# hannesweisbach/channelcoding

Hardware: AMD Instinct MI355X
Metric: decoded frames/sec (coded bits/sec = value x 255), BCH(255,231) min-sum, batch=2^20 (higher is better)
Workload: dtype f32

## Files before the change

channelcoding_amd/csrc/cc_internal.hpp:

```cpp
#pragma once
#include <hip/hip_runtime.h>

#include <cstdint>
#include <memory>
#include <mutex>
#include <string>
#include <vector>

#include "../../include/channelcoding_amd.h"
#include "galois.hpp"

namespace ccamd {

struct MinSumGeometry {
  int W = 64, C = 4, frames_per_wave = 1, KW = 1;
};

struct MinSumParams {
  int n, K, KW;
  int variant;
  int stop_rule;
  unsigned iterations;
  float alpha_f;
  float beta_f;
// ... 111 lines not shown
  bool scms;
  int np = 0;
  int gap[4] = {0, 0, 0, 0};
};
const DiagGeometry *diag_geometry(const CodeTables &t);
std::vector<uint16_t> build_diag_table(const CodeTables &t, int D, int W, int np = 0, const int *gap = nullptr);
size_t minsum_diag_lds_bytes(const DiagGeometry &g);
MinSumParams minsum_params(const cc_code *code);
bool minsum_shortcuts_enabled();
bool minsum_diag_supported(const cc_code *code);
int launch_minsum_diag_compact(const cc_code *code, uint32_t *d_ctl, uint32_t *d_pool, unsigned cap, const float *d_llr,
                               uint8_t *d_hard, uint16_t *d_iters, int32_t *d_status, hipStream_t stream);
std::string minsum_diag_name(const cc_code *code);
int launch_minsum_diag(const cc_code *code, const MinSumParams &p, const float *d_llr, const uint16_t *d_er,
                       const uint32_t *d_er_off, uint8_t *d_hard, float *d_L, uint16_t *d_iters, int32_t *d_status,
                       size_t B, hipStream_t stream);
bool algebraic_long_needed(const cc_code *code, bool erasures);
int launch_algebraic_long(const cc_code *code, bool float_in, const void *d_in, const uint16_t *d_er,
                          const uint32_t *d_er_off, uint8_t *d_out, int32_t *d_nerr, int32_t *d_status, size_t B,
                          hipStream_t stream);
int launch_algebraic(const cc_code *code, bool float_in, const void *d_in, const uint16_t *d_er,
                     const uint32_t *d_er_off, uint8_t *d_out, int32_t *d_nerr, int32_t *d_status, size_t B,
                     hipStream_t stream);
bool algebraic_chunk_supported(const cc_code *code, bool erasures);
int launch_algebraic_chunk(const cc_code *code, bool float_in, const void *d_in, const uint16_t *d_er,
                           const uint32_t *d_er_off, uint8_t *d_out, int32_t *d_nerr, int32_t *d_status, size_t B,
                           hipStream_t stream, int il = 1);
int launch_chase(const cc_code *code, const float *d_llr, unsigned p, uint8_t *d_out, int32_t *d_nerr, float *d_metric,
                 int32_t *d_status, size_t B, hipStream_t stream);
int chase_frames_per_wave(const cc_code *code, unsigned p, bool soft);
int launch_chase_soft(const cc_code *code, const float *d_llr, unsigned p, float beta, uint8_t *d_out, float *d_ext,
                      int32_t *d_nerr, float *d_metric, int32_t *d_status, size_t B, hipStream_t stream);
int launch_gmd(const cc_code *code, const uint8_t *d_words, const float *d_rel, unsigned m, uint8_t *d_out, int32_t *d_nerr,
               float *d_metric, int32_t *d_status, size_t B, hipStream_t stream);
bool bitslice_supported(const cc_code *code);
int launch_bitslice_syndromes(const cc_code *code, bool float_in, const void *d_in, uint8_t *d_out, uint8_t *d_synd, size_t B,
                              hipStream_t stream, int il = 1);
bool bitslice_encode_supported(const cc_code *code);
int launch_bitslice_encode(const cc_code *code, const uint8_t *d_msg, uint8_t *d_cw, size_t B, hipStream_t stream, int il = 1);
int launch_bitslice_chien(const void *d_lamp, void *d_masks, size_t B, bool long_locators, hipStream_t stream);
int launch_bitslice_roots_transpose(const void *d_masks, void *d_rootsT, size_t B, hipStream_t stream);
constexpr uint32_t kLogZero = 512;
int launch_chunk_bm(const cc_code *code, const uint8_t *d_synd, const uint16_t *d_er, const uint32_t *d_er_off,
                    uint16_t *d_llg, uint16_t *d_meta, unsigned long long *d_mask, uint8_t *d_lamp, int ncoef,
                    uint32_t *d_nleft, int32_t *d_nerr, int32_t *d_status, size_t B, hipStream_t stream);
int algebraic_route(const cc_code *code, size_t B, bool erasures);
bool planes_small_call(const cc_code *code, size_t B);
int launch_pgz_erasures(const cc_code *code, const uint8_t *d_in, const uint16_t *d_er, const uint32_t *d_er_off,
                        uint8_t *d_out, int32_t *d_nerr, int32_t *d_status, size_t B, hipStream_t stream);
constexpr int diag_variant_part(int variant, int parts) {
  const int order = variant == CC_ALG_MS ? 0 : variant == CC_ALG_NMS ? 1 : variant == CC_ALG_OMS ? 2
                  : variant == CC_ALG_SCMS2 ? 3 : variant == CC_ALG_SCMS1 ? 4 : 5;
  return order % parts;
}

int launch_wide_correct(const cc_code *code, const uint16_t *d_in, const uint16_t *d_er, const uint32_t *d_off,
                        uint16_t *d_out, int32_t *d_nerr, int32_t *d_status, size_t B, hipStream_t stream);
int launch_wide_pgz_erasures(const cc_code *code, const uint16_t *d_in, const uint16_t *d_er, const uint32_t *d_off,
                        uint16_t *d_out, int32_t *d_nerr, int32_t *d_status, size_t B, hipStream_t stream);
int launch_wide_encode(const cc_code *code, const uint16_t *d_msg, uint16_t *d_cw, size_t B, hipStream_t stream);
int launch_wide_extract(const cc_code *code, const uint16_t *d_cw, uint16_t *d_msg, size_t B, hipStream_t stream);
std::vector<uint8_t> build_parity_table(const Field &f, const CodeTables &t);
int launch_encode(const cc_code *code, const uint8_t *d_msg, uint8_t *d_cw, size_t B, hipStream_t stream);
int launch_encode_bits(const cc_code *code, const uint8_t *d_msg, uint8_t *d_cw, size_t B, hipStream_t stream);
int launch_extract(const cc_code *code, const uint8_t *d_cw, uint8_t *d_msg, size_t B, hipStream_t stream);
int launch_pack_bits(const void *d_sym, int width, size_t n, uint8_t *d_packed, size_t B, hipStream_t stream);
int launch_unpack_bits(const uint8_t *d_packed, size_t n, void *d_sym, int width, size_t B, hipStream_t stream);
bool packed_native_supported(const cc_code *code, size_t B);
int launch_packed_correct(const cc_code *code, const uint8_t *d_in, uint8_t *d_out, int32_t *d_nerr, int32_t *d_status,
                          size_t B, hipStream_t stream);
bool packed_long_supported(const cc_code *code, size_t B);
int launch_packed_long_correct(const cc_code *code, const uint8_t *d_in, uint8_t *d_out, int32_t *d_nerr, int32_t *d_status,
                               size_t B, hipStream_t stream);
bool packed_encode_native(const cc_code *code);
bool packed_extract_native(const cc_code *code);
int launch_packed_encode(const cc_code *code, const uint8_t *d_msg, uint8_t *d_cw, size_t B, hipStream_t stream);
int launch_packed_extract(const cc_code *code, const uint8_t *d_cw, uint8_t *d_msg, size_t B, hipStream_t stream);
constexpr size_t kInterleaveMax = 256;
constexpr size_t kInterleaveNativeMax = 16;
int launch_interleave(const void *d_in, int width, size_t n, size_t I, void *d_out, size_t B, bool to_interleaved,
                      hipStream_t stream);
bool interleaved_native_supported(const cc_code *code, size_t B, size_t I, bool erasures);
bool interleaved_encode_native(const cc_code *code, size_t I);
bool interleaved_extract_native(const cc_code *code, size_t I);
int launch_interleaved_extract(const cc_code *code, const void *d_cw, void *d_msg, size_t B, size_t I, hipStream_t stream);
int mc_run(cc_code *code, double ebno_db, uint64_t seed, uint64_t first_frame, size_t frames, int random_codewords,
           uint64_t *d_counters, hipStream_t stream);
int mc_run_chase(cc_code *code, unsigned p, double ebno_db, uint64_t seed, uint64_t first_frame, size_t frames,
                 int random_codewords, uint64_t *d_counters, hipStream_t stream);
int mc_run_gmd(cc_code *code, unsigned m, double ebno_db, uint64_t seed, uint64_t first_frame, size_t frames,
               int random_codewords, uint64_t *d_counters, hipStream_t stream);
int mc_awgn_symbols(cc_code *code, double ebno_db, uint64_t seed, uint64_t first_frame, size_t frames, int random_codewords,
                    uint8_t *d_words, float *d_rel, uint8_t *d_sent, hipStream_t stream);
int mc_awgn(cc_code *code, double ebno_db, uint64_t seed, uint64_t first_frame, size_t frames, int random_codewords,
            float *d_llr, uint8_t *d_sent, hipStream_t stream);
int mc_run_discrete(cc_code *code, double p_error, double p_erasure, uint64_t seed, uint64_t first_frame, size_t frames,
                    int random_codewords, uint64_t *d_counters, hipStream_t stream);
int mc_discrete(cc_code *code, double p_error, double p_erasure, uint64_t seed, uint64_t first_frame, size_t frames,
                int random_codewords, uint8_t *d_recv, uint16_t *d_erasures, uint32_t *d_erasure_offsets,
                uint8_t *d_sent, hipStream_t stream);
int mc_run_burst(cc_code *code, const cc_burst_channel &ch, uint64_t seed, uint64_t first_frame, size_t frames,
                 int random_codewords, uint64_t *d_counters, hipStream_t stream);
int mc_burst(cc_code *code, const cc_burst_channel &ch, uint64_t seed, uint64_t first_frame, size_t frames,
             int random_codewords, uint8_t *d_recv, uint8_t *d_sent, uint8_t *d_state, hipStream_t stream);
int mc_run_burst_erasure(cc_code *code, const cc_burst_channel &ch, const cc_burst_detector &det, uint64_t seed,
                         uint64_t first_frame, size_t frames, int random_codewords, uint64_t *d_counters,
// ... 23 lines not shown
```

channelcoding_amd/csrc/minsum_diag.hip:

```cpp
#include "minsum_diag_impl.hpp"

#include <algorithm>
#include <cstdlib>

namespace ccamd {

using DiagLaunch = int (*)(const cc_code *, const MinSumParams &, const float *, const uint16_t *, const uint32_t *,
                           uint8_t *, float *, uint16_t *, int32_t *, size_t, hipStream_t);
#define CC_PART_DECL(NAME, I)                                                                                        \
  int launch_minsum_diag_##NAME##_p##I(const cc_code *, const MinSumParams &, const float *, const uint16_t *,       \
                                       const uint32_t *, uint8_t *, float *, uint16_t *, int32_t *, size_t, hipStream_t);
#define CC_PARTS_1(M, NAME) M(NAME, 0)
#define CC_PARTS_2(M, NAME) CC_PARTS_1(M, NAME) M(NAME, 1)
#define CC_PARTS_3(M, NAME) CC_PARTS_2(M, NAME) M(NAME, 2)
#define CC_PARTS_6(M, NAME) CC_PARTS_3(M, NAME) M(NAME, 3) M(NAME, 4) M(NAME, 5)
#define GEO(NAME, N, KK, W, DD, LL, CC, OO, SC, PA, LK, PP) CC_PARTS_##PP(CC_PART_DECL, NAME)
#include "minsum_diag_geos.inc"
#undef GEO
namespace {
struct DiagEntry {
  DiagGeometry geo;
  int parts;
  DiagLaunch launch[6];
};
// ... 139 lines not shown
      grp[g].push_back(grp[D - 1].back());
      grp[D - 1].pop_back();
    }
  const size_t real_last = grp[D - 1].size();
  auto group_cost = [&](const std::vector<unsigned> &g) {
    int cnt[16] = {0}, mx = 0, sq = 0;
    for (unsigned s : g) ++cnt[s % 16];
    for (int c : cnt) {
      mx = c > mx ? c : mx;
      sq += c * c;
    }
    return mx * 1000 + sq;
  };
  bool improved = true;
  while (improved) {
    improved = false;
    for (int a = 0; a < D && !improved; ++a)
      for (int b = a + 1; b < D && !improved; ++b)
        for (size_t x = 0; x < grp[a].size() && !improved; ++x)
          for (size_t y = 0; y < grp[b].size() && !improved; ++y) {
            const int before = group_cost(grp[a]) + group_cost(grp[b]);
            std::swap(grp[a][x], grp[b][y]);
            if (group_cost(grp[a]) + group_cost(grp[b]) < before)
              improved = true;
            else
              std::swap(grp[a][x], grp[b][y]);
          }
  }
  std::vector<uint16_t> out(static_cast<size_t>(D) * W, 0xFFFFu);
  for (int g = 0; g < D; ++g)
    for (size_t l = 0; l < grp[g].size(); ++l) out[g * W + l] = static_cast<uint16_t>(grp[g][l]);
  (void)real_last;
  return out;
}

bool minsum_diag_supported(const cc_code *code) {
  if (code->d_diag == nullptr || code->desc.iterations == 0) return false;
  const int alg = code->desc.algorithm;
  const DiagGeometry *geo = diag_geometry(code->tab);
  if (!geo) return false;
  if (alg == CC_ALG_SCMS1) return true;
  if (alg == CC_ALG_SCMS2) return geo->scms;
  if (alg != CC_ALG_MS && alg != CC_ALG_NMS && alg != CC_ALG_OMS && alg != CC_ALG_2DNMS) return false;
  if (alg == CC_ALG_OMS && !(code->desc.beta >= 0.0)) return false;
  const float a = static_cast<float>(code->desc.alpha);
  if ((alg == CC_ALG_NMS || alg == CC_ALG_2DNMS) && !(a == a && a - a == 0.0f)) return false;
  return diag_geometry(code->tab) != nullptr;
}


std::string minsum_diag_name(const cc_code *code) {
  const DiagGeometry *g = diag_geometry(code->tab);
  if (!g) return "minsum_diag_kernel";
  return "minsum_diag_kernel<K=" + std::to_string(g->k) + ",D=" + std::to_string(g->D) + ",LPF=" +
         std::to_string(g->LPF) + ",row-pipelined>";
}

size_t minsum_diag_lds_bytes(const DiagGeometry &g) {
  const bool partial = g.w != static_cast<unsigned>(g.LPF * g.D);
  const size_t fpw = 64 / g.LPF, rc = static_cast<size_t>(g.LPF) * g.CPL + (partial ? 48 : (g.LPF == 8 && g.CPL == 8 ? 8 : 16));
  return 4 * (fpw * rc * 8 + (fpw / 2) * rc * 8) + 256 * 4 +
         4 * static_cast<size_t>(g.CPL) * 256;
}


namespace {

__global__ void __launch_bounds__(256)
twopass_gather_kernel(const uint32_t *__restrict__ ctl, unsigned sample, unsigned cap, const uint32_t *__restrict__ list,
                      const float *__restrict__ llr, float *__restrict__ llr2, int n) {
  if (!two_pass_in_effect(ctl, sample, cap)) return;
  const unsigned long long cnt = ctl[1];
  const int lane = threadIdx.x & 63;
  const unsigned long long nwaves = static_cast<unsigned long long>(gridDim.x) * 4;
  for (unsigned long long k = static_cast<unsigned long long>(blockIdx.x) * 4 + (threadIdx.x >> 6); k < cnt; k += nwaves) {
    const float *src = llr + static_cast<unsigned long long>(list[k]) * n;
    float *dst = llr2 + k * n;
    for (int j = lane; j < n; j += 64) dst[j] = src[j];
  }
}
__global__ void __launch_bounds__(256)
twopass_scatter_kernel(const uint32_t *__restrict__ ctl, unsigned sample, unsigned cap, const uint32_t *__restrict__ list,
                       const uint8_t *__restrict__ hard2, const uint16_t *__restrict__ iters2,
                       const int32_t *__restrict__ status2, uint8_t *__restrict__ hard, uint16_t *__restrict__ iters,
                       int32_t *__restrict__ status, int n) {
  if (!two_pass_in_effect(ctl, sample, cap)) return;
  const unsigned long long cnt = ctl[1];
  const int lane = threadIdx.x & 63;
  const unsigned long long nwaves = static_cast<unsigned long long>(gridDim.x) * 4;
  for (unsigned long long k = static_cast<unsigned long long>(blockIdx.x) * 4 + (threadIdx.x >> 6); k < cnt; k += nwaves) {
    const unsigned long long f = list[k];
    for (int j = lane; j < n; j += 64) hard[f * n + j] = hard2[k * n + j];
    if (lane == 0) {
      if (iters) iters[f] = iters2[k];
      if (status) status[f] = status2[k];
    }
  }
}

bool two_pass_enabled() { return minsum_shortcuts_enabled(); }

int launch_two_pass(const cc_code *code, const DiagEntry *e, const MinSumParams &p, const float *d_llr, uint8_t *d_hard,
                    uint16_t *d_iters, int32_t *d_status, size_t B, hipStream_t stream) {
  const size_t n = code->tab.n, cap = B / 4, sample = 4096;
  auto up = [](size_t v) { return (v + 255) & ~static_cast<size_t>(255); };
  constexpr size_t max_runs = 4, o_pool = 256, pool_bytes = POOL_WORDS * 4;
  const size_t o_list = o_pool + (max_runs + 2) * pool_bytes, o_llr = o_list + up(cap * 4), o_hard = o_llr + up(cap * n * 4),
               o_it = o_hard + up(cap * n), o_st = o_it + up(cap * 2), total = o_st + up(cap * 4);
// ... 108 lines not shown
```

channelcoding_amd/csrc/minsum_diag_impl.hpp:

```cpp
#pragma once
#include <cstdio>
#include <cstdlib>
#include <type_traits>
#include <utility>

#include "cc_internal.hpp"
#include "wave_ops.hpp"


namespace ccamd {
namespace {



template <int... Is, typename F>
__device__ __forceinline__ void static_for_impl(std::integer_sequence<int, Is...>, F &&f) {
  (f(std::integral_constant<int, Is>{}), ...);
}
template <int N, typename F>
__device__ __forceinline__ void static_for(F &&f) {
  static_for_impl(std::make_integer_sequence<int, N>{}, static_cast<F &&>(f));
}
template <int... Gs>
struct PairGaps {
// ... 58 lines not shown
  v = xor_stage<0x4E>(v);
  v = xor_stage<0x141>(v);
  return LPF == 16 ? xor_stage<0x140>(v) : v;
}
template <int LPF>
__device__ __forceinline__ uint32_t group_or(uint32_t v) {
  v = or_stage<0xB1>(v);
  v = or_stage<0x4E>(v);
  v = or_stage<0x141>(v);
  return LPF == 16 ? or_stage<0x140>(v) : v;
}

__device__ __forceinline__ void transposed_reduce4(const uint32_t (&a1)[4], const uint32_t (&a2)[4], const uint32_t (&sg)[4],
                                                   uint32_t &z1, uint32_t &z2, uint32_t &zs) {
  uint32_t x1, x2, xs, y1, y2, ys, h, t, h2, t2;
  asm volatile(
      "s_nop 1\n\t"
      "v_max_u32_dpp %[h], %[a10], %[a10] row_ror:8 row_mask:0xf bank_mask:0x3\n\t"
      "v_max_u32_dpp %[h], %[a12], %[a12] row_ror:8 row_mask:0xf bank_mask:0xc\n\t"
      "v_min_u32_dpp %[x1], %[a10], %[a10] row_ror:8 row_mask:0xf bank_mask:0x3\n\t"
      "v_min_u32_dpp %[x1], %[a12], %[a12] row_ror:8 row_mask:0xf bank_mask:0xc\n\t"
      "v_min_u32_dpp %[t], %[a20], %[a20] row_ror:8 row_mask:0xf bank_mask:0x3\n\t"
      "v_min_u32_dpp %[t], %[a22], %[a22] row_ror:8 row_mask:0xf bank_mask:0xc\n\t"
      "v_xor_b32_dpp %[xs], %[s0], %[s0] row_ror:8 row_mask:0xf bank_mask:0x3\n\t"
      "v_xor_b32_dpp %[xs], %[s2], %[s2] row_ror:8 row_mask:0xf bank_mask:0xc\n\t"
      "v_min_u32 %[x2], %[t], %[h]\n\t"
      "v_max_u32_dpp %[h2], %[a11], %[a11] row_ror:8 row_mask:0xf bank_mask:0x3\n\t"
      "v_max_u32_dpp %[h2], %[a13], %[a13] row_ror:8 row_mask:0xf bank_mask:0xc\n\t"
      "v_min_u32_dpp %[y1], %[a11], %[a11] row_ror:8 row_mask:0xf bank_mask:0x3\n\t"
      "v_min_u32_dpp %[y1], %[a13], %[a13] row_ror:8 row_mask:0xf bank_mask:0xc\n\t"
      "v_min_u32_dpp %[t2], %[a21], %[a21] row_ror:8 row_mask:0xf bank_mask:0x3\n\t"
      "v_min_u32_dpp %[t2], %[a23], %[a23] row_ror:8 row_mask:0xf bank_mask:0xc\n\t"
      "v_xor_b32_dpp %[ys], %[s1], %[s1] row_ror:8 row_mask:0xf bank_mask:0x3\n\t"
      "v_xor_b32_dpp %[ys], %[s3], %[s3] row_ror:8 row_mask:0xf bank_mask:0xc\n\t"
      "v_min_u32 %[y2], %[t2], %[h2]\n\t"
      "v_max_u32_dpp %[h], %[x1], %[x1] row_shl:4 row_mask:0xf bank_mask:0x5\n\t"
      "v_min_u32_dpp %[z1], %[x1], %[x1] row_shl:4 row_mask:0xf bank_mask:0x5\n\t"
      "v_min_u32_dpp %[t], %[x2], %[x2] row_shl:4 row_mask:0xf bank_mask:0x5\n\t"
      "v_xor_b32_dpp %[zs], %[xs], %[xs] row_shl:4 row_mask:0xf bank_mask:0x5\n\t"
      "v_max_u32_dpp %[h], %[y1], %[y1] row_shr:4 row_mask:0xf bank_mask:0xa\n\t"
      "v_min_u32_dpp %[z1], %[y1], %[y1] row_shr:4 row_mask:0xf bank_mask:0xa\n\t"
      "v_min_u32_dpp %[t], %[y2], %[y2] row_shr:4 row_mask:0xf bank_mask:0xa\n\t"
      "v_xor_b32_dpp %[zs], %[ys], %[ys] row_shr:4 row_mask:0xf bank_mask:0xa\n\t"
      "v_min_u32 %[z2], %[t], %[h]\n\t"
      "v_max_u32_dpp %[h], %[z1], %[z1] quad_perm:[1,0,3,2] row_mask:0xf bank_mask:0xf\n\t"
      "v_min_u32_dpp %[z1], %[z1], %[z1] quad_perm:[1,0,3,2] row_mask:0xf bank_mask:0xf\n\t"
      "v_xor_b32_dpp %[zs], %[zs], %[zs] quad_perm:[1,0,3,2] row_mask:0xf bank_mask:0xf\n\t"
      "v_mov_b32_dpp %[t], %[z2] quad_perm:[1,0,3,2] row_mask:0xf bank_mask:0xf\n\t"
      "v_min3_u32 %[z2], %[h], %[z2], %[t]\n\t"
      "v_max_u32_dpp %[h], %[z1], %[z1] quad_perm:[2,3,0,1] row_mask:0xf bank_mask:0xf\n\t"
      "v_min_u32_dpp %[z1], %[z1], %[z1] quad_perm:[2,3,0,1] row_mask:0xf bank_mask:0xf\n\t"
      "v_xor_b32_dpp %[zs], %[zs], %[zs] quad_perm:[2,3,0,1] row_mask:0xf bank_mask:0xf\n\t"
      "v_mov_b32_dpp %[t], %[z2] quad_perm:[2,3,0,1] row_mask:0xf bank_mask:0xf\n\t"
      "v_min3_u32 %[z2], %[h], %[z2], %[t]"
      : [x1] "=&v"(x1), [x2] "=&v"(x2), [xs] "=&v"(xs), [y1] "=&v"(y1), [y2] "=&v"(y2), [ys] "=&v"(ys), [h] "=&v"(h),
        [t] "=&v"(t), [h2] "=&v"(h2), [t2] "=&v"(t2), [z1] "=&v"(z1), [z2] "=&v"(z2), [zs] "=&v"(zs)
      : [a10] "v"(a1[0]), [a11] "v"(a1[1]), [a12] "v"(a1[2]), [a13] "v"(a1[3]), [a20] "v"(a2[0]), [a21] "v"(a2[1]),
        [a22] "v"(a2[2]), [a23] "v"(a2[3]), [s0] "v"(sg[0]), [s1] "v"(sg[1]), [s2] "v"(sg[2]), [s3] "v"(sg[3]));
}

__device__ __forceinline__ float min_abs2(float a, float b) {
  float r;
  asm("v_min_f32_e64 %0, |%1|, |%2|" : "=v"(r) : "v"(a), "v"(b));
  return r;
}
__device__ __forceinline__ float max_abs2(float a, float b) {
  float r;
  asm("v_max_f32_e64 %0, |%1|, |%2|" : "=v"(r) : "v"(a), "v"(b));
  return r;
}
__device__ __forceinline__ float min_abs1(float a, float q) {
  float r;
  asm("v_min_f32_e64 %0, %1, |%2|" : "=v"(r) : "v"(a), "v"(q));
  return r;
}
__device__ __forceinline__ float med3_abs3(float a, float b, float c) {
  float r;
  asm("v_med3_f32 %0, |%1|, |%2|, |%3|" : "=v"(r) : "v"(a), "v"(b), "v"(c));
  return r;
}
__device__ __forceinline__ float min3_abs3(float a, float b, float c) {
  float r;
  asm("v_min3_f32 %0, |%1|, |%2|, |%3|" : "=v"(r) : "v"(a), "v"(b), "v"(c));
  return r;
}
__device__ __forceinline__ float med3_abs23(float a, float b, float c) {
  float r;
  asm("v_med3_f32 %0, %1, |%2|, |%3|" : "=v"(r) : "v"(a), "v"(b), "v"(c));
  return r;
}
__device__ __forceinline__ float min3_abs23(float a, float b, float c) {
  float r;
  asm("v_min3_f32 %0, %1, |%2|, |%3|" : "=v"(r) : "v"(a), "v"(b), "v"(c));
  return r;
}
__device__ __forceinline__ float med3_abs1(float a1, float q, float a2) {
  float r;
  asm("v_med3_f32 %0, %1, |%2|, %3" : "=v"(r) : "v"(a1), "v"(q), "v"(a2));
  return r;
}

__device__ __forceinline__ uint32_t shift_in_is_zero(uint32_t acc, float t) {
  asm("v_cmp_eq_f32 vcc, 0, %1\n\tv_addc_co_u32 %0, vcc, %0, %0, vcc" : "+v"(acc) : "v"(t) : "vcc");
  return acc;
}

__device__ __forceinline__ int signum(float v) { return (0.0f < v) - (v < 0.0f); }
template <int VARIANT>
__device__ __forceinline__ float self_correct(float tmp, float q_old) {
  if constexpr (VARIANT == CC_ALG_SCMS1) {
    const int so = signum(q_old);
    return (so == 0 || so == signum(tmp)) ? tmp : 0.0f;
  } else {
    return (tmp * q_old > 0.0f) ? tmp : 0.5f * (tmp + q_old);
  }
}

template <int VARIANT>
__device__ __forceinline__ float horizontal(float m, float alpha_f, double beta_d) {
  if constexpr (VARIANT == CC_ALG_NMS || VARIANT == CC_ALG_2DNMS) {
    return __fmul_rn(alpha_f, m);
  } else if constexpr (VARIANT == CC_ALG_OMS) {
    const double a = static_cast<double>(m) - beta_d;
    return static_cast<float>((a < 0.0) ? 0.0 : a);
  } else {
    return m;
  }
}

template <int K, int D, int VARIANT, int RB, int LPF, int CPL, int OCC, bool PARTIAL, typename PG = PairGaps<>,
          bool SINGLE = false, bool CHAIN = false>
__global__ void __launch_bounds__(256, OCC)
minsum_diag_kernel(MinSumParams p, const uint16_t *__restrict__ diag_s, const uint32_t *__restrict__ colbits,
                   const float *__restrict__ llr, const uint16_t *__restrict__ er, const uint32_t *__restrict__ er_off,
                   uint8_t *__restrict__ hard, float *__restrict__ Lout, uint16_t *__restrict__ iters_out,
                   int32_t *__restrict__ status_out, unsigned long long B) {
  static_assert(K % RB == 0 && K <= 32, "row batching");
  if (p.gate == 1 && !two_pass_sampled(p)) return;
  if (p.dual && two_pass_in_effect(p.ctl, p.sample, p.list_cap)) {
    llr = p.llr2;
    hard = p.hard2;
    Lout = nullptr;
    iters_out = p.iters2;
    status_out = p.status2;
    B = p.ctl[1] < p.list_cap ? p.ctl[1] : p.list_cap;
  }
  static_assert(LPF == 8 || LPF == 16, "a frame occupies half or all of a 16-lane DPP row");
  static_assert(2 * PG::NP <= D && !(PARTIAL && PG::NP > 0), "paired slots");
  static_assert(!CHAIN || PG::NP == 0 || (PG::gap(0) == 1 && PG::gap(PG::NP - 1) == 1), "links are gap-1 pairs");
  constexpr int NLK = CHAIN ? PG::NP : 0;
  constexpr int FPW = 64 / LPF;
  constexpr int RC = LPF * CPL + (PARTIAL ? 48 : (LPF == 8 && CPL == 8 ? 8 : 16));
  extern __shared__ __attribute__((aligned(16))) char smem[];
  constexpr int CY_BYTES = FPW * RC * 8, CN_BYTES = (FPW / 2) * RC * 8;
  constexpr int WAVE_BYTES = CY_BYTES + (SINGLE ? 0 : CN_BYTES);
  const int lane = threadIdx.x & 63, wid = threadIdx.x >> 6;
  const int fl = lane / LPF, lam = lane & (LPF - 1);
  char *cy_base = smem + wid * WAVE_BYTES;
  char *cn_lane = cy_base + CY_BYTES + ((fl >> 1) - fl) * RC * 8 + (fl & 1) * 4;
  uint32_t *cbits = reinterpret_cast<uint32_t *>(smem + 4 * WAVE_BYTES);
  char *stg = smem + 4 * WAVE_BYTES + 1024 + wid * (CPL * 256);
  const uint32_t stg_lds = __builtin_amdgcn_readfirstlane(static_cast<uint32_t>(reinterpret_cast<size_t>(stg)));
  cbits[threadIdx.x] = colbits[threadIdx.x];
  constexpr bool POOL = !SINGLE && LPF == 16;
  __shared__ unsigned wg_next;
  if (!POOL && threadIdx.x == 0) wg_next = 2 * 4 * (64 / LPF);
  __syncthreads();

  const int n = p.n;
  int aCY[D];
#pragma unroll
  for (int d = 0; d < D; ++d) aCY[d] = (fl * RC + diag_s[d * LPF + lam]) * 8;
  float pen = 0.0f;
  uint32_t sgn_keep = 0xFFFFFFFFu;
  if constexpr (PARTIAL) {
    if (diag_s[(D - 1) * LPF + lam] == 0xFFFFu) {
      aCY[D - 1] = (fl * RC + LPF * CPL + 16) * 8;
      pen = 3.402823466e+38f;
      sgn_keep = 0u;
    }
  }
  const int col0 = fl * RC + lam;
  const bool oddf = SINGLE && (fl & 1);
#ifndef CC_EXP_O0_B32
// ... 98 lines not shown
          const int j = lam + LPF * c;
          if (j < n) {
            uint32_t m0_save;
            asm volatile("s_mov_b32 %0, m0\n\ts_mov_b32 m0, %2\n\ts_nop 0\n\tglobal_load_lds_dword %1, off\n\ts_mov_b32 m0, %0"
                         : "=&s"(m0_save) : "v"(src + j), "s"(stg_lds + c * 256) : "memory");
          }
        }
      }
    }
  };
  const char *stg_full = stg + fl * LPF * 16 + lam * 4;
  const char *stg_tail = stg + NF * 1024 + fl * LPF * 16 + (lam - n + 4 * LPF) * 4;
  auto staged = [&](int c) -> float {
    if constexpr (X4) {
      if (c < 4 * NF) return *reinterpret_cast<const float *>(stg_full + (c / 4) * 1024 + (c % 4) * 4 * LPF);
      return *reinterpret_cast<const float *>(stg_tail + 4 * LPF * c);
    } else {
      return *reinterpret_cast<const float *>(stg + c * 256 + lane * 4);
    }
  };
  auto setup = [&](unsigned long long f) {
#pragma unroll
    for (int c = 0; c < CPL; ++c) {
      float y = staged(c) + 0.0f;
      if (c == CPL - 1 && lam + LPF * c >= n) y = 0.0f;
      *reinterpret_cast<float2 *>(cy_base + (col0 + LPF * c) * 8) = make_cell(0.0f, y);
    }
    if (er_off != nullptr) {
      for (uint32_t e = er_off[f]; e < er_off[f + 1]; ++e) {
        const int pos = er[e];
        if ((pos & (LPF - 1)) == lam) *reinterpret_cast<float *>(cy_base + (fl * RC + pos) * 8 + y_off) = 0.0f;
      }
    }
    if constexpr (!SINGLE && !QONLY) static_for<K>([&](auto I) { static_for<D>([&](auto Dd) { R[I][Dd] = 0.0f; }); });
    if constexpr (KEEPQ) static_for<K>([&](auto I) { static_for<D>([&](auto Dd) { Q[I][Dd] = 0.0f; }); });
    if constexpr (QONLY)
      for (int r = lam; r < K; r += LPF) my_rows[r] = make_uint2(0u, 0u);
    if constexpr (BITS1) static_for<NW>([&](auto Wd) { SW[Wd] = 0u; ZW[Wd] = 0xFFFFFFFFu; });
  };

#pragma unroll
  for (int c = 0; c < CPL; ++c)
    if constexpr (!SINGLE) *reinterpret_cast<float *>(cn_lane + (col0 + LPF * c) * 8) = 0.0f;
  if (active) {
    stage(frame);
    asm volatile("s_waitcnt vmcnt(0)" ::: "memory");
    setup(frame);
    stage(nextf);
    if (POOL && PREDRAW && lam == 0) opd = draw();
  }

  while (__any(active)) {
    constexpr bool PREFETCH = !(BITS1 && K * D >= 160) && !SINGLE;
#ifdef CC_EXP_TRED
    constexpr bool TRED = LPF == 16 && K % 4 == 0 && !SINGLE;
#else
    constexpr bool TRED = false;
#endif
    constexpr bool EARLY_PF = TRED && PREFETCH;
    float2 cyq[D];
    float2 carry_cy[NLK ? NLK : 1];
    float carry_sum[NLK ? NLK : 1];
    auto fetch = [&](auto IC) {
      constexpr int row = decltype(IC)::value;
      if constexpr (QONLY) rsq = my_rows[row];
      static_for<D>([&](auto DD) {
        constexpr int d = DD;
        if constexpr (d < 2 * NLK && (d & 1) == 0 && row >= 1) {
          cyq[d] = carry_cy[d / 2];
          return;
        }
#ifdef CC_EXP_NO_CYR
        asm volatile("" : "=v"(cyq[d].x), "=v"(cyq[d].y));
#else
#ifdef CC_EXP_O0_B32
        if constexpr (SINGLE) {
          const int at = aCY[slot_base<PG>(d)] + 8 * (row + slot_gap<PG>(d));
          cyq[d].x = *reinterpret_cast<const float *>(cy_base + at + (4 - y_off));
          cyq[d].y = *reinterpret_cast<const float *>(cy_base + at + y_off);
          return;
        }
#endif
        cyq[d] = *reinterpret_cast<const float2 *>(cy_base + aCY[slot_base<PG>(d)] + 8 * (row + slot_gap<PG>(d)));
#endif
      });
    };
    float Tloc[D];
    auto row_front = [&](auto IR, uint32_t &o1, uint32_t &o2, uint32_t &os) {
      constexpr int i = decltype(IR)::value;
      if constexpr (!PREFETCH) fetch(IR);
      [[maybe_unused]] auto wget = [&](auto DD) -> float {
        if constexpr (SINGLE) return Tloc[DD];
        else if constexpr (QONLY) return Q[i][DD];
        else return R[i][DD];
      };
      auto wset = [&](auto DD, float v) {
        if constexpr (SINGLE) Tloc[DD] = v;
        else if constexpr (!QONLY) R[i][DD] = v;
      };
      [[maybe_unused]] const float old_hi = u2f(rsq.y & 0x7FFFFFFFu);
      [[maybe_unused]] uint32_t old_Y = (rsq.x ^ rsq.y);
      if constexpr (QONLY) asm volatile("" : "+v"(old_Y));
      {
        float a1 = 0.0f, a2 = (D == 1) ? 3.402823466e+38f : 0.0f;
        uint32_t s = 0;
        uint32_t qs[D];
        float mag[D], qv[D];
        uint32_t keep = 0;
        constexpr int wi = BITS1 ? i / RPW : 0, sh = BITS1 ? (i % RPW) * D : 0;
        if constexpr (BITS1) {
          uint32_t tw = 0, tz = 0;
          static_for<D>([&](auto DD) {
            constexpr int d = DD;
            const float t = (cyq[d].x - R[i][d]) + cyq[d].y;
            R[i][d] = t;
            tw = __builtin_amdgcn_alignbit(tw, f2u(t), 31);
            tz = shift_in_is_zero(tz, t);
          });
          constexpr uint32_t field = ((D == 32 ? 0u : (1u << D)) - 1u) << sh;
          const uint32_t tws = tw << sh, tzs = tz << sh;
// ... 63 lines not shown
            a1 = RAW ? min3_abs23(a1, mag[d - 1], mag[d]) : __builtin_fminf(__builtin_fminf(a1, mag[d - 1]), mag[d]);
            a2 = __builtin_fminf(a2, md);
          } else if constexpr (d == D - 1 && d >= 3 && (d & 1) == 1) {
            a2 = RAW ? med3_abs1(a1, mag[d], a2) : __builtin_amdgcn_fmed3f(a1, mag[d], a2);
            a1 = RAW ? min_abs1(a1, mag[d]) : __builtin_fminf(a1, mag[d]);
          }
        });
        s = qs[0];
        static_for<(D - 1) / 2>([&](auto T) {
          s = static_cast<uint32_t>(__builtin_amdgcn_bitop3_b32(static_cast<int>(s), static_cast<int>(qs[1 + 2 * T]),
                                                                static_cast<int>(qs[2 + 2 * T]), 0x96));
        });
        if constexpr ((D - 1) % 2) s ^= qs[D - 1];
        o1 = f2u(a1);
        o2 = f2u(a2);
        os = s;
      }
      if constexpr (!EARLY_PF) {
        static_for<NLK>([&](auto P) { carry_cy[P] = cyq[2 * P + 1]; });
        if constexpr (PREFETCH && i + 1 < K) fetch(std::integral_constant<int, i + 1>{});
      }
    };
    auto row_cn = [&](auto IR, float (&cn)[D]) {
      constexpr int i = decltype(IR)::value;
      static_for<D>([&](auto DD) {
        constexpr int d = DD;
        if constexpr (d < 2 * NLK && (d & 1) == 0 && i >= 1)
          cn[d] = carry_sum[d / 2];
        else if constexpr (SINGLE)
          cn[d] = cell_cs(cyq[d]);
        else
#ifdef CC_EXP_NO_CNR
          asm volatile("" : "=v"(cn[d]));
#else
          cn[d] = *reinterpret_cast<const float *>(cn_lane + aCY[slot_base<PG>(d)] + 8 * (i + slot_gap<PG>(d)));
#endif
      });
    };
    auto row_back = [&](auto IR, uint32_t m1v, uint32_t m2v, uint32_t sg0, float (&cn)[D]) {
      constexpr int i = decltype(IR)::value;
      float rt[QONLY ? D : 1];
      bool made = false;
      (void)made;
      [[maybe_unused]] auto wget = [&](auto DD) -> float {
        if constexpr (SINGLE) return Tloc[DD];
        else if constexpr (QONLY) return made ? rt[DD] : Q[i][DD];
        else return R[i][DD];
      };
      auto wset = [&](auto DD, float v) {
        if constexpr (SINGLE) Tloc[DD] = v;
        else if constexpr (QONLY) rt[DD] = v;
        else R[i][DD] = v;
      };
      asm volatile("" : "+v"(sg0));
      const uint32_t sign31 = sg0 & 0x80000000u;
      if constexpr (VARIANT == CC_ALG_MS || VARIANT == CC_ALG_SCMS1 || VARIANT == CC_ALG_SCMS2) {
        uint32_t Y = (m1v ^ m2v) | sign31;
#ifndef CC_EXP_BITOP3_POST
        asm volatile("" : "+v"(Y));
#endif
        const float hi = u2f(m2v);
        static_for<D>([&](auto DD) {
          wset(DD, u2f(f2u(__builtin_amdgcn_fmed3f(wget(DD), -hi, hi)) ^ Y));
        });
      } else {
        const uint32_t H1 = f2u(horizontal<VARIANT>(u2f(m1v), p.alpha_f, p.beta_d));
        const uint32_t H2 = f2u(horizontal<VARIANT>(u2f(m2v), p.alpha_f, p.beta_d));
        static_for<D>([&](auto DD) {
          const uint32_t mag = (__builtin_fabsf(wget(DD)) == u2f(m1v)) ? H2 : H1;
          wset(DD, u2f(xad(mag, sign31, f2u(wget(DD)) & 0x80000000u)));
        });
      }
      made = true;
      if constexpr (QONLY) {
        if (lam == 0) my_rows[i] = make_uint2(m1v, m2v | sign31);
      }
      float sum[D];
      static_for<D>([&](auto DD) {
        constexpr int d = D - 1 - DD;
        sum[d] = cn[d] + wget(std::integral_constant<int, d>{});
      });
      __builtin_amdgcn_sched_barrier(0);
      static_for<D>([&](auto DD) {
        constexpr int d = DD;
        if constexpr (d < 2 * NLK && (d & 1) == 1 && i + 1 < K)
          carry_sum[d / 2] = sum[d];
        else if constexpr (SINGLE)
          *reinterpret_cast<float *>(cy_base + aWR[slot_base<PG>(d)] + 8 * (i + slot_gap<PG>(d))) = sum[d];
        else
#ifdef CC_EXP_NO_CNW
          asm volatile("" ::"v"(sum[d]));
#else
          *reinterpret_cast<float *>(cn_lane + aCY[slot_base<PG>(d)] + 8 * (i + slot_gap<PG>(d))) = sum[d];
#endif
      });
      asm volatile("" ::: "memory");
    };
    if constexpr (PREFETCH) fetch(std::integral_constant<int, 0>{});
    if constexpr (TRED) {
      static_for<K / 4>([&](auto IG) {
        constexpr int g = IG;
        uint32_t a1[4], a2[4], sg[4];
        static_for<4>([&](auto J) { row_front(std::integral_constant<int, 4 * g + J>{}, a1[J], a2[J], sg[J]); });
        uint32_t z1, z2, zs;
        transposed_reduce4(a1, a2, sg, z1, z2, zs);
        uint32_t M1[4], M2[4], SG[4];
        static_for<4>([&](auto J) {
          constexpr int pat = 0x13 | (J << 7);
          M1[J] = static_cast<uint32_t>(__builtin_amdgcn_ds_swizzle(static_cast<int>(z1), pat));
          M2[J] = static_cast<uint32_t>(__builtin_amdgcn_ds_swizzle(static_cast<int>(z2), pat));
          SG[J] = static_cast<uint32_t>(__builtin_amdgcn_ds_swizzle(static_cast<int>(zs), pat));
        });
        static_for<4>([&](auto J) {
          float cn[D];
          row_cn(std::integral_constant<int, 4 * g + J>{}, cn);
          row_back(std::integral_constant<int, 4 * g + J>{}, M1[J], M2[J], SG[J], cn);
        });
      });
    } else {
      static_for<K>([&](auto IR) {
        uint32_t m1[1], m2[1], sg[1];
        row_front(IR, m1[0], m2[0], sg[0]);
        float cn[D];
        row_cn(IR, cn);
#ifndef CC_EXP_NO_REDUCE
        row_allreduce<1, LPF>(m1, m2, sg);
#endif
        row_back(IR, m1[0], m2[0], sg[0], cn);
      });
    }

    uint32_t acc = 0;
    auto stop_scan = [&](auto ORC) {
      float cnv[CPL], yc[CPL];
      uint32_t cb[CPL];
#pragma unroll
      for (int c = 0; c < CPL; ++c) {
        if constexpr (SINGLE) {
          const float2 cy = *reinterpret_cast<const float2 *>(cy_base + (col0 + LPF * c) * 8);
          cnv[c] = cy.x;
          yc[c] = cy.y;
        } else {
          cnv[c] = *reinterpret_cast<const float *>(cn_lane + (col0 + LPF * c) * 8);
          yc[c] = *reinterpret_cast<const float *>(cy_base + (col0 + LPF * c) * 8 + 4);
        }
        cb[c] = cbits[lam + LPF * c];
      }
      asm volatile("" ::: "memory");
#pragma unroll
      for (int c = 0; c < CPL; ++c) {
        const int m = static_cast<int>(f2u(cnv[c] + yc[c])) >> 31;
        if constexpr (decltype(ORC)::value)
          acc = static_cast<uint32_t>(__builtin_amdgcn_bitop3_b32(static_cast<int>(acc), m, static_cast<int>(cb[c]), 0xF8));
        else
          acc = static_cast<uint32_t>(__builtin_amdgcn_bitop3_b32(static_cast<int>(acc), m, static_cast<int>(cb[c]), 0x78));
      }
      if constexpr (!SINGLE) {
#pragma unroll
        for (int c = 0; c < CPL; ++c) {
          *reinterpret_cast<float *>(cy_base + (col0 + LPF * c) * 8) = cnv[c];
          *reinterpret_cast<float *>(cn_lane + (col0 + LPF * c) * 8) = 0.0f;
        }
      }
    };
    bool ok;
    if (SINGLE && p.stop_rule == CC_STOP_AS_SHIPPED) {
      ok = true;
    } else if (p.stop_rule == CC_STOP_PUBLISHED) {
      stop_scan(std::true_type{});
      ok = group_or<LPF>(acc) == 0;
    } else {
// ... 80 lines not shown
    } else {
      ++it;
    }
  }
  asm volatile("s_waitcnt vmcnt(0)" ::: "memory");
}

}

namespace {

template <int K, int D, int LPF, int CPL, int OCC, bool SCMS = false, bool PARTIAL = false, typename PG = PairGaps<>,
          bool CHAIN = false, int PARTS = 1, int PART = 0>
int launch_diag_geometry(const cc_code *code, const MinSumParams &p, const float *d_llr, const uint16_t *d_er,
                         const uint32_t *d_er_off, uint8_t *d_hard, float *d_L, uint16_t *d_iters, int32_t *d_status,
                         size_t B, hipStream_t stream) {
  constexpr int RB = 1;
  constexpr bool Q_ONLY_2 = 2 * K * D + 64 > 256, Q_ONLY_1 = K * D >= 160 && OCC >= 2;
  constexpr int OCC_S = Q_ONLY_2 ? OCC : (2 * K * D + 64 <= 128) ? 4 : (2 * K * D + 64 <= 168) ? 3 : 2;
  constexpr int FPW = 64 / LPF;
  if (!(code->tab.n > static_cast<unsigned>(LPF * (CPL - 1)) && code->tab.n <= static_cast<unsigned>(LPF * CPL))) {
    set_last_error("minsum_diag: only the last owned column of a lane may lie beyond the frame");
    return CC_ERR_UNSUPPORTED;
  }
  if (p.pool == nullptr || B >= (1ull << 32)) {
    set_last_error("minsum_diag: no frame pool, or more than 2^32 frames in one call");
    return CC_ERR_UNSUPPORTED;
  }
  const DiagGeometry g{0, 0, PARTIAL ? 1u : static_cast<unsigned>(LPF * D), D, LPF, CPL, SCMS};
  const size_t lds = minsum_diag_lds_bytes(g);
  const unsigned long long blocks_needed = (B + 4 * FPW - 1) / (4 * FPW);
  constexpr size_t ords_bytes = LPF == 16 ? 4 * FPW * sizeof(uint2) : 0;
  unsigned long long per_cu = (160 * 1024) / (lds + ords_bytes);
  const unsigned long long occ = p.variant == CC_ALG_SCMS2 ? static_cast<unsigned long long>(OCC_S) : OCC;
  if ((p.variant == CC_ALG_SCMS2 && Q_ONLY_2) || (p.variant == CC_ALG_SCMS1 && Q_ONLY_1))
    per_cu = (160 * 1024) / (lds + ords_bytes + 4 * FPW * K * sizeof(uint2));
  if (per_cu > occ) per_cu = occ;
  const unsigned long long max_grid = static_cast<unsigned long long>(code->num_cus) * per_cu;
  const int grid = static_cast<int>(blocks_needed < max_grid ? blocks_needed : max_grid);
  const unsigned long long Bq = B;
  hipError_t e = hipSuccess;
  const bool single = p.stop_rule == CC_STOP_AS_SHIPPED || p.iterations == 1 || p.first_pass != 0;
  constexpr size_t rc_cols = static_cast<size_t>(LPF) * CPL + (PARTIAL ? 48 : (LPF == 8 && CPL == 8 ? 8 : 16));
  const size_t lds_s = lds - 4 * (FPW / 2) * rc_cols * 8;
  unsigned long long per_cu_s = (160 * 1024) / lds_s;
  if (per_cu_s > 8) per_cu_s = 8;
  const unsigned long long max_grid_s = static_cast<unsigned long long>(code->num_cus) * per_cu_s;
  const int grid_s = static_cast<int>(blocks_needed < max_grid_s ? blocks_needed : max_grid_s);
#define CC_LAUNCH_S(V, O, S)                                                                                       \
  {                                                                                                                \
    const size_t lds_k = (S) ? lds_s : lds;                                                                        \
    const int grid_k = (S) ? grid_s : grid;                                                                        \
    e = hipFuncSetAttribute(                                                                                       \
        reinterpret_cast<const void *>(&minsum_diag_kernel<K, D, V, RB, LPF, CPL, O, PARTIAL, PG, S, CHAIN>),      \
        hipFuncAttributeMaxDynamicSharedMemorySize, static_cast<int>(lds_k));                                     \
    if (e == hipSuccess)                                                                                           \
      hipLaunchKernelGGL((minsum_diag_kernel<K, D, V, RB, LPF, CPL, O, PARTIAL, PG, S, CHAIN>), dim3(grid_k), dim3(256), lds_k, \
                         stream, p, code->d_diag, code->d_colbits, d_llr, d_er, d_er_off, d_hard, d_L, d_iters,    \
                         d_status, Bq);                                                                            \
  }
#define CC_LAUNCH(V, O)                                                                                            \
  {                                                                                                                \
    if constexpr (diag_variant_part(V, PARTS) != PART) e = hipErrorInvalidValue;                                   \
    else if (single) CC_LAUNCH_S(V, OCC, true) else CC_LAUNCH_S(V, O, false)                                       \
  }
  switch (p.variant) {
    case CC_ALG_MS: CC_LAUNCH(CC_ALG_MS, OCC) break;
    case CC_ALG_NMS: CC_LAUNCH(CC_ALG_NMS, OCC) break;
    case CC_ALG_OMS: CC_LAUNCH(CC_ALG_OMS, OCC) break;
    case CC_ALG_2DNMS: CC_LAUNCH(CC_ALG_2DNMS, OCC) break;
    case CC_ALG_SCMS1:
      CC_LAUNCH(CC_ALG_SCMS1, OCC)
      break;
    case CC_ALG_SCMS2:
      if constexpr (SCMS) CC_LAUNCH(CC_ALG_SCMS2, OCC_S) else e = hipErrorInvalidValue;
      break;
    default: e = hipErrorInvalidValue;
  }
#undef CC_LAUNCH
#undef CC_LAUNCH_S
  if (e == hipSuccess) e = hipGetLastError();
  if (e != hipSuccess) return hip_fail(e, "minsum_diag kernel launch");
  return CC_OK;
}

}

}
```

Before: 68.31 million.

## Enable four-row transposed reduction with DPP row broadcast in min-sum diag kernel

Turns on by default the previously experimental path that processes four check rows per transposed DPP reduction for the K=24, D=7, LPF=16 geometry with plain min-sum variants. The path is used for non-single launches only. The ds_swizzle broadcasts are replaced by DPP row_newbcast moves, and for plain MS the sign/magnitude word is precombined before the broadcast to save a broadcast and some ALU work. An optional pipelined body overlaps the next group's front with the current group's back. The change adds register pressure and a reversed column order, and it risks spills or wrong results if row_newbcast behaves unexpectedly, which a new probe program checks.

Result: faster. 71.40 million, median of 6 (+4.5%).

```diff
diff --git a/channelcoding_amd/csrc/cc_internal.hpp b/channelcoding_amd/csrc/cc_internal.hpp
--- a/channelcoding_amd/csrc/cc_internal.hpp
+++ b/channelcoding_amd/csrc/cc_internal.hpp
@@ -187,6 +187,15 @@
   const int order = variant == CC_ALG_MS ? 0 : variant == CC_ALG_NMS ? 1 : variant == CC_ALG_OMS ? 2
                   : variant == CC_ALG_SCMS2 ? 3 : variant == CC_ALG_SCMS1 ? 4 : 5;
   return order % parts;
+}
+
+enum DiagRowBody { DIAG_ROWS_BUTTERFLY = 0, DIAG_ROWS_FOUR = 1, DIAG_ROWS_FOUR_PIPELINED = 2 };
+#ifndef CC_DIAG_FOUR_ROW_BODY
+#define CC_DIAG_FOUR_ROW_BODY 1
+#endif
+constexpr int diag_row_body(int K, int D, int LPF, int variant) {
+  const bool plain = variant == CC_ALG_MS || variant == CC_ALG_NMS || variant == CC_ALG_OMS || variant == CC_ALG_2DNMS;
+  return (K == 24 && D == 7 && LPF == 16 && plain) ? CC_DIAG_FOUR_ROW_BODY : DIAG_ROWS_BUTTERFLY;
 }
 
 int launch_wide_correct(const cc_code *code, const uint16_t *d_in, const uint16_t *d_er, const uint32_t *d_off,
diff --git a/channelcoding_amd/csrc/minsum_diag.hip b/channelcoding_amd/csrc/minsum_diag.hip
--- a/channelcoding_amd/csrc/minsum_diag.hip
+++ b/channelcoding_amd/csrc/minsum_diag.hip
@@ -215,8 +215,9 @@
 std::string minsum_diag_name(const cc_code *code) {
   const DiagGeometry *g = diag_geometry(code->tab);
   if (!g) return "minsum_diag_kernel";
-  return "minsum_diag_kernel<K=" + std::to_string(g->k) + ",D=" + std::to_string(g->D) + ",LPF=" +
-         std::to_string(g->LPF) + ",row-pipelined>";
+  const int body = diag_row_body(static_cast<int>(g->k), g->D, g->LPF, code->desc.algorithm);
+  return "minsum_diag_kernel<K=" + std::to_string(g->k) + ",D=" + std::to_string(g->D) + ",LPF=" + std::to_string(g->LPF) +
+         (body == DIAG_ROWS_FOUR_PIPELINED ? ",four-row-pipelined>" : body == DIAG_ROWS_FOUR ? ",four-row>" : ",row-pipelined>");
 }
 
 size_t minsum_diag_lds_bytes(const DiagGeometry &g) {
diff --git a/channelcoding_amd/csrc/minsum_diag_impl.hpp b/channelcoding_amd/csrc/minsum_diag_impl.hpp
--- a/channelcoding_amd/csrc/minsum_diag_impl.hpp
+++ b/channelcoding_amd/csrc/minsum_diag_impl.hpp
@@ -134,11 +134,17 @@
       "v_min_u32_dpp %[z1], %[z1], %[z1] quad_perm:[2,3,0,1] row_mask:0xf bank_mask:0xf\n\t"
       "v_xor_b32_dpp %[zs], %[zs], %[zs] quad_perm:[2,3,0,1] row_mask:0xf bank_mask:0xf\n\t"
       "v_mov_b32_dpp %[t], %[z2] quad_perm:[2,3,0,1] row_mask:0xf bank_mask:0xf\n\t"
-      "v_min3_u32 %[z2], %[h], %[z2], %[t]"
+      "v_min3_u32 %[z2], %[h], %[z2], %[t]\n\t"
+      "s_nop 1"
       : [x1] "=&v"(x1), [x2] "=&v"(x2), [xs] "=&v"(xs), [y1] "=&v"(y1), [y2] "=&v"(y2), [ys] "=&v"(ys), [h] "=&v"(h),
         [t] "=&v"(t), [h2] "=&v"(h2), [t2] "=&v"(t2), [z1] "=&v"(z1), [z2] "=&v"(z2), [zs] "=&v"(zs)
       : [a10] "v"(a1[0]), [a11] "v"(a1[1]), [a12] "v"(a1[2]), [a13] "v"(a1[3]), [a20] "v"(a2[0]), [a21] "v"(a2[1]),
         [a22] "v"(a2[2]), [a23] "v"(a2[3]), [s0] "v"(sg[0]), [s1] "v"(sg[1]), [s2] "v"(sg[2]), [s3] "v"(sg[3]));
+}
+
+template <int J>
+__device__ __forceinline__ uint32_t bank_bcast(uint32_t v) {
+  return static_cast<uint32_t>(__builtin_amdgcn_mov_dpp(static_cast<int>(v), 0x150 + 4 * J, 0xF, 0xF, true));
 }
 
 __device__ __forceinline__ float min_abs2(float a, float b) {
@@ -211,7 +217,7 @@
 }
 
 template <int K, int D, int VARIANT, int RB, int LPF, int CPL, int OCC, bool PARTIAL, typename PG = PairGaps<>,
-          bool SINGLE = false, bool CHAIN = false>
+          bool SINGLE = false, bool CHAIN = false, int BODY = DIAG_ROWS_BUTTERFLY>
 __global__ void __launch_bounds__(256, OCC)
 minsum_diag_kernel(MinSumParams p, const uint16_t *__restrict__ diag_s, const uint32_t *__restrict__ colbits,
                    const float *__restrict__ llr, const uint16_t *__restrict__ er, const uint32_t *__restrict__ er_off,
@@ -416,11 +422,10 @@
 
   while (__any(active)) {
     constexpr bool PREFETCH = !(BITS1 && K * D >= 160) && !SINGLE;
-#ifdef CC_EXP_TRED
-    constexpr bool TRED = LPF == 16 && K % 4 == 0 && !SINGLE;
-#else
-    constexpr bool TRED = false;
-#endif
+    constexpr bool TRED = BODY != DIAG_ROWS_BUTTERFLY;
+    static_assert(!TRED || (LPF == 16 && K % 4 == 0 && !SINGLE && !NEEDQ),
+                  "four rows per reduction: a frame per DPP row, whole row groups, plain variants (the self-correcting ones spill)");
+    constexpr bool READY = TRED && VARIANT == CC_ALG_MS;
     constexpr bool EARLY_PF = TRED && PREFETCH;
     float2 cyq[D];
     float2 carry_cy[NLK ? NLK : 1];
@@ -429,7 +434,7 @@
       constexpr int row = decltype(IC)::value;
       if constexpr (QONLY) rsq = my_rows[row];
       static_for<D>([&](auto DD) {
-        constexpr int d = DD;
+        constexpr int d = TRED ? D - 1 - DD : DD;
         if constexpr (d < 2 * NLK && (d & 1) == 0 && row >= 1) {
           cyq[d] = carry_cy[d / 2];
           return;
@@ -599,10 +604,10 @@
         else if constexpr (QONLY) rt[DD] = v;
         else R[i][DD] = v;
       };
-      asm volatile("" : "+v"(sg0));
+      if constexpr (!READY) asm volatile("" : "+v"(sg0));
       const uint32_t sign31 = sg0 & 0x80000000u;
       if constexpr (VARIANT == CC_ALG_MS || VARIANT == CC_ALG_SCMS1 || VARIANT == CC_ALG_SCMS2) {
-        uint32_t Y = (m1v ^ m2v) | sign31;
+        uint32_t Y = READY ? m1v : (m1v ^ m2v) | sign31;
 #ifndef CC_EXP_BITOP3_POST
         asm volatile("" : "+v"(Y));
 #endif
@@ -645,25 +650,46 @@
     };
     if constexpr (PREFETCH) fetch(std::integral_constant<int, 0>{});
     if constexpr (TRED) {
-      static_for<K / 4>([&](auto IG) {
-        constexpr int g = IG;
+      constexpr int NG = K / 4;
+      uint32_t ZA[NG], ZB[NG], ZC[READY ? 1 : NG];
+      auto fronts = [&](auto IG) {
+        constexpr int g = decltype(IG)::value;
         uint32_t a1[4], a2[4], sg[4];
         static_for<4>([&](auto J) { row_front(std::integral_constant<int, 4 * g + J>{}, a1[J], a2[J], sg[J]); });
         uint32_t z1, z2, zs;
         transposed_reduce4(a1, a2, sg, z1, z2, zs);
-        uint32_t M1[4], M2[4], SG[4];
-        static_for<4>([&](auto J) {
-          constexpr int pat = 0x13 | (J << 7);
-          M1[J] = static_cast<uint32_t>(__builtin_amdgcn_ds_swizzle(static_cast<int>(z1), pat));
-          M2[J] = static_cast<uint32_t>(__builtin_amdgcn_ds_swizzle(static_cast<int>(z2), pat));
-          SG[J] = static_cast<uint32_t>(__builtin_amdgcn_ds_swizzle(static_cast<int>(zs), pat));
-        });
+        if constexpr (READY) {
+          ZA[g] = (z1 ^ z2) | (zs & 0x80000000u);
+          ZB[g] = z2;
+        } else {
+          ZA[g] = z1;
+          ZB[g] = z2;
+          ZC[g] = zs;
+        }
+      };
+      auto backs = [&](auto IG) {
+        constexpr int g = decltype(IG)::value;
         static_for<4>([&](auto J) {
           float cn[D];
           row_cn(std::integral_constant<int, 4 * g + J>{}, cn);
-          row_back(std::integral_constant<int, 4 * g + J>{}, M1[J], M2[J], SG[J], cn);
+          const uint32_t b0 = bank_bcast<J>(ZA[g]), b1 = bank_bcast<J>(ZB[g]);
+          uint32_t b2 = 0;
+          if constexpr (!READY) b2 = bank_bcast<J>(ZC[g]);
+          row_back(std::integral_constant<int, 4 * g + J>{}, b0, b1, b2, cn);
         });
-      });
+      };
+      if constexpr (BODY == DIAG_ROWS_FOUR_PIPELINED) {
+        fronts(std::integral_constant<int, 0>{});
+        static_for<NG>([&](auto IG) {
+          if constexpr (IG + 1 < NG) fronts(std::integral_constant<int, IG + 1>{});
+          backs(IG);
+        });
+      } else {
+        static_for<NG>([&](auto IG) {
+          fronts(IG);
+          backs(IG);
+        });
+      }
     } else {
       static_for<K>([&](auto IR) {
         uint32_t m1[1], m2[1], sg[1];
@@ -850,11 +876,14 @@
     const size_t lds_k = (S) ? lds_s : lds;                                                                        \
     const int grid_k = (S) ? grid_s : grid;                                                                        \
     e = hipFuncSetAttribute(                                                                                       \
-        reinterpret_cast<const void *>(&minsum_diag_kernel<K, D, V, RB, LPF, CPL, O, PARTIAL, PG, S, CHAIN>),      \
+        reinterpret_cast<const void *>(&minsum_diag_kernel<K, D, V, RB, LPF, CPL, O, PARTIAL, PG, S, CHAIN,        \
+                                                           (S) ? DIAG_ROWS_BUTTERFLY : diag_row_body(K, D, LPF, V)>), \
         hipFuncAttributeMaxDynamicSharedMemorySize, static_cast<int>(lds_k));                                     \
     if (e == hipSuccess)                                                                                           \
-      hipLaunchKernelGGL((minsum_diag_kernel<K, D, V, RB, LPF, CPL, O, PARTIAL, PG, S, CHAIN>), dim3(grid_k), dim3(256), lds_k, \
-                         stream, p, code->d_diag, code->d_colbits, d_llr, d_er, d_er_off, d_hard, d_L, d_iters,    \
+      hipLaunchKernelGGL((minsum_diag_kernel<K, D, V, RB, LPF, CPL, O, PARTIAL, PG, S, CHAIN,                        \
+                                             (S) ? DIAG_ROWS_BUTTERFLY : diag_row_body(K, D, LPF, V)>),               \
+                         dim3(grid_k), dim3(256), lds_k, stream, p, code->d_diag, code->d_colbits, d_llr, d_er,    \
+                         d_er_off, d_hard, d_L, d_iters,                                                           \
                          d_status, Bq);                                                                            \
   }
 #define CC_LAUNCH(V, O)                                                                                            \
diff --git a/profiles/ubench/row_newbcast_probe.hip b/profiles/ubench/row_newbcast_probe.hip
--- /dev/null
+++ b/profiles/ubench/row_newbcast_probe.hip
@@ -0,0 +1,37 @@
+#include <hip/hip_runtime.h>
+#include <cstdio>
+__global__ void k(unsigned *o) {
+  const unsigned v = threadIdx.x;
+  unsigned r[8];
+  asm volatile(
+      "s_nop 1\n\t"
+      "v_mov_b32_dpp %0, %4 row_newbcast:0 row_mask:0xf bank_mask:0xf\n\t"
+      "v_mov_b32_dpp %1, %4 row_newbcast:4 row_mask:0xf bank_mask:0xf\n\t"
+      "v_mov_b32_dpp %2, %4 row_newbcast:8 row_mask:0xf bank_mask:0xf\n\t"
+      "v_mov_b32_dpp %3, %4 row_newbcast:12 row_mask:0xf bank_mask:0xf"
+      : "=&v"(r[0]), "=&v"(r[1]), "=&v"(r[2]), "=&v"(r[3])
+      : "v"(v));
+  r[4] = static_cast<unsigned>(__builtin_amdgcn_mov_dpp(static_cast<int>(v), 0x150, 0xF, 0xF, true));
+  r[5] = static_cast<unsigned>(__builtin_amdgcn_mov_dpp(static_cast<int>(v), 0x154, 0xF, 0xF, true));
+  r[6] = static_cast<unsigned>(__builtin_amdgcn_mov_dpp(static_cast<int>(v), 0x158, 0xF, 0xF, true));
+  r[7] = static_cast<unsigned>(__builtin_amdgcn_mov_dpp(static_cast<int>(v), 0x15C, 0xF, 0xF, true));
+  for (int j = 0; j < 8; ++j) o[j * 64 + threadIdx.x] = r[j];
+}
+int main() {
+  unsigned *o, h[8 * 64];
+  if (hipMalloc(&o, sizeof(h)) != hipSuccess) { printf("no device memory\n"); return 2; }
+  (void)hipMemset(o, 0xFF, sizeof(h));
+  k<<<1, 64>>>(o);
+  if (hipMemcpy(h, o, sizeof(h), hipMemcpyDeviceToHost) != hipSuccess) { printf("copy failed\n"); return 2; }
+  int bad_total = 0;
+  for (int j = 0; j < 8; ++j) {
+    const unsigned n = 4 * (j % 4);
+    int bad = 0;
+    for (unsigned t = 0; t < 64; ++t) bad += h[j * 64 + t] != 16 * (t / 16) + n;
+    printf("%s row_newbcast:%-2u lanes 0 / 15 / 16 / 37 / 63 read %u / %u / %u / %u / %u; %d of 64 lanes differ from 16 (lane / 16) + %u\n",
+           j < 4 ? "asm    " : "builtin", n, h[j * 64], h[j * 64 + 15], h[j * 64 + 16], h[j * 64 + 37], h[j * 64 + 63], bad, n);
+    bad_total += bad;
+  }
+  printf(bad_total ? "FAIL\n" : "PASS: every lane of a DPP row reads lane n of its own row\n");
+  return bad_total ? 1 : 0;
+}
```
